# ArjunTeh/AdjointNonlinearRayTracing

Measured on AMD Instinct MI355X. Metric: ray-steps/sec (fwd+adjoint), 256^3 RIF grid, 1M rays x 512 steps, higher is better.
Workload: dtype f32

## Files before the change

### adjointnonlinearraytracing_amd/_lib.py

```python
from __future__ import annotations

import ctypes as C
import os
from typing import Optional

_HERE = os.path.dirname(os.path.abspath(__file__))
LIB_PATH = os.environ.get("DRRT_HIP_LIB") or os.path.join(_HERE, "libdrrt_hip.so")

FLAG_NONE = 0
FLAG_SORT_RAYS = 1
FLAG_CORRECTED_H = 2
FLAG_NO_ZERO = 4
FLAG_DIRECT_ATOMICS = 8
FLAG_DEBUG_COUNTERS = 16
FLAG_PAIR_GRID = 64
FLAG_PAIR_REUSE = 128
FLAG_QUAD_GRID, FLAG_QUAD_REUSE = FLAG_PAIR_GRID, FLAG_PAIR_REUSE
FLAG_Q16_POS_ONLY = 0x200000
FLAG_STATIC_WINDOW = 0x400000
FLAG_CHORD_KEY = 0x800000
FLAG_RING_WINDOW = 0x1000000
FLAG_DISPATCH_IN_ORDER = 0x2000000
FLAG_RING_SPARSE, FLAG_RING_GENERAL, FLAG_RING_DIRECT = 0x4000000, 0x8000000, 0x10000000
ADAM_MASK_BOUNDARY, ADAM_CLAMP_MIN = 1, 2

ERR_RES_MISMATCH, ERR_BAD_RES, ERR_ARG, ERR_HIP = -1, -2, -3, -4


class Stats(C.Structure):
    _fields_ = [("ray_steps", C.c_ulonglong), ("n_failed", C.c_ulonglong),
                ("iters", C.c_uint), ("reserved", C.c_uint)]


STATS_BYTES = C.sizeof(Stats)

_vp, _f, _sz, _u, _ll, _i = C.c_void_p, C.c_float, C.c_size_t, C.c_uint, C.c_longlong, C.c_int
_d = C.c_double
_tail = [_vp, _vp, _sz, _u, _vp]


def _sensor_signatures():
    e = [_vp, _f]
    splat = ([_i, _f, _vp, _u, _vp], [_i, _f, _vp, _vp, _vp, _vp])
    families = {
        "splat": ([_sz, _vp, _vp] + e, 4) + splat,
        "far_splat": ([_sz, _vp] + e, 2) + splat,
        "tex_get": ([_sz, _vp, _vp], 4, [_vp, _i, _f, _i, _vp, _vp], [_vp, _i, _f, _i, _vp, _vp, _vp, _vp]),
    }
    return {f"drrt_sensor_{family}{dframe}{bwd}_f32": (_i, rays + [_vp] * (1 if dframe else host) + tails[bool(bwd)])
            for family, (rays, host, *tails) in families.items() for dframe in ("", "_dframe") for bwd in ("", "_bwd")}


SIGNATURES = {
    "drrt_workspace_bytes": (_sz, [_sz, _u]),
    "drrt_workspace_bytes_grid": (_sz, [_sz, _ll, _u]),
    "drrt_last_error": (C.c_char_p, []),
    "drrt_version": (C.c_char_p, []),
    "drrt_trace_f32": (_i, [_vp, _ll, _vp, _sz, _vp, _vp, _f, _f, _vp, _vp] + _tail),
    "drrt_trace_f16io": (_i, [_vp, _ll, _vp, _sz, _vp, _vp, _f, _f, _vp, _vp] + _tail),
    "drrt_backtrace_f16io": (_i, [_vp, _ll, _vp, _sz, _vp, _vp, _vp, _vp, _f, _f, _vp] + _tail),
    "drrt_trace_q16io": (_i, [_vp, _ll, _vp, _sz, _vp, _vp, _f, _f, _vp, _vp] + _tail),
    "drrt_backtrace_q16io": (_i, [_vp, _ll, _vp, _sz, _vp, _vp, _vp, _vp, _f, _f, _vp] + _tail),
    "drrt_q16_params": (_i, [_vp, _f, _vp]),
    "drrt_q16_encode": (_i, [_vp, _f, _sz, _vp, _vp, _vp, _vp, _vp]),
    "drrt_q16_decode": (_i, [_vp, _f, _sz, _vp, _vp, _vp, _vp, _vp]),
    "drrt_trace_pln_f32": (_i, [_vp, _ll, _vp, _sz, _vp, _vp, _vp, _vp, _f, _f, _vp, _vp, _vp] + _tail),
    "drrt_trace_target_f32": (_i, [_vp, _ll, _vp, _sz, _vp, _vp, _vp, _f, _f, _vp, _vp, _vp] + _tail),
    "drrt_trace_sdf_f32": (_i, [_vp, _vp, _ll, _vp, _sz, _vp, _vp, _f, _f, _vp, _vp] + _tail),
    "drrt_trace_cable_f32": (_i, [_vp, _sz, _f, _f, _sz, _vp, _vp, _vp, _f, _vp, _vp, _vp] + _tail),
    "drrt_backtrace_f32": (_i, [_vp, _ll, _vp, _sz, _vp, _vp, _vp, _vp, _f, _f, _vp] + _tail),
    "drrt_backtrace_rays_f32": (_i, [_vp, _ll, _vp, _sz, _vp, _vp, _vp, _vp, _vp, _vp, _vp, _f, _f, _vp, _vp] + _tail),
    "drrt_trace_opl_f32": (_i, [_vp, _ll, _vp, _sz, _vp, _vp, _f, _f, _vp, _vp, _vp, _vp] + _tail),
    "drrt_backtrace_opl_f32": (_i, [_vp, _ll, _vp, _sz, _vp, _vp, _vp, _vp, _vp, _vp, _vp, _vp, _f, _f, _vp, _vp, _vp] + _tail),
    "drrt_trace_field_f32": (_i, [_vp, _vp, _ll, _vp, _sz, _vp, _vp, _f, _f, _vp, _vp, _vp, _vp] + _tail),
    "drrt_backtrace_field_f32": (_i, [_vp, _vp, _ll, _vp, _sz, _vp, _vp, _vp, _vp, _vp, _vp, _vp, _vp, _f, _f, _vp, _vp, _vp, _vp] + _tail),
    "drrt_trace_emission_f32": (_i, [_vp, _vp, _vp, _ll, _vp, _sz, _vp, _vp, _f, _f, _vp, _vp, _vp, _vp, _vp] + _tail),
    "drrt_backtrace_emission_f32": (_i, [_vp, _vp, _vp, _ll, _vp, _sz, _vp, _vp, _vp, _vp, _vp, _vp, _vp, _vp, _vp, _vp, _f, _f,
                                         _vp, _vp, _vp, _vp, _vp] + _tail),
    "drrt_backtrace_chunk_state_bytes": (_sz, [_sz]),
    "drrt_backtrace_max_steps": (_i, [_vp, _f, _f]),
    "drrt_backtrace_chunk_f32": (_i, [_vp, _ll, _vp, _sz, _vp, _vp, _vp, _vp, _f, _f, _vp] + _tail + [_vp, _sz, _i, _i, _vp]),
    "drrt_backtrace_sdf_f32": (_i, [_vp, _vp, _ll, _vp, _sz, _vp, _vp, _vp, _vp, _f, _f, _vp] + _tail),
    "drrt_backtrace_cable_f32": (_i, [_vp, _sz, _f, _f, _sz, _vp, _vp, _vp, _vp, _f, _vp] + _tail),
    "drrt_backtrace_cable_rays_f32": (_i, [_vp, _sz, _f, _f, _sz, _vp, _vp, _vp, _vp, _vp, _f, _vp, _vp] + _tail),
    "drrt_backtrace_pln_rays_f32": (_i, [_vp, _ll, _vp, _sz, _vp, _vp, _vp, _vp, _vp, _vp, _f, _f, _vp, _vp] + _tail),
    "drrt_backtrace_sdf_rays_f32": (_i, [_vp, _vp, _ll, _vp, _sz, _vp, _vp, _vp, _vp, _f, _f, _vp, _vp] + _tail),
    "drrt_backtrace_target_rays_f32": (_i, [_vp, _ll, _vp, _sz, _vp, _vp, _vp, _vp, _vp, _vp, _f, _f, _vp, _vp] + _tail),
    **_sensor_signatures(),
    "drrt_rays_to_plane_f32": (_i, [_sz, _vp, _vp, _vp, _vp, _i, _vp, _vp]),
    "drrt_rays_to_plane_bwd_f32": (_i, [_sz, _vp, _vp, _vp, _vp, _i, _vp, _vp, _vp, _vp]),
    "drrt_upres_volume_f32": (_i, [_vp, _vp, _vp, _vp, _vp]),
    "drrt_adam_step_f32": (_i, [_vp, _vp, _vp, _vp, _vp, _d, _d, _d, _d, _d, _d, _d, _u, _vp]),
    "drrt_gen_workspace_bytes": (_sz, [_i, _i, _i, _i]),
    "drrt_gen_rays_f32": (_i, [_i, _vp, _vp, _i, _i, _i, _i, _d, _d, _i, _i, _vp, _d, _vp, _vp, _vp, _vp, _vp, _sz, _vp]),
    "drrt_gen_cone_rays_f32": (_i, [_vp, _vp, _i, _i, _i, _i, _d, _d, _d, _vp, _d, _vp, _vp, _vp, _vp, _vp, _sz, _vp]),
    "drrt_last_order": (_vp, [_vp]),
    "drrt_set_order_hint": (None, [_vp, _sz]),
    "drrt_order_hint_pending": (_sz, []),
    "drrt_last_steps": (_vp, [_vp]),
    "drrt_set_step_hint": (None, [_vp, _sz]),
    "drrt_last_bundle_counters": (_vp, []),
    "drrt_ring_threshold_pct": (_i, []),
    "drrt_ring_long_threshold_permille": (_i, []),
    "drrt_ring_direct_threshold_pct": (_i, []),
    "drrt_profile_begin": (_i, [_i]),
    "drrt_profile_collect": (_i, [_vp, _vp, _i]),
    "drrt_profile_end": (None, []),
}

PROF_NAMES = {1: "trace", 2: "backtrace", 3: "sort", 4: "zero", 5: "quad", 6: "backtrace_rays",
              7: "backtrace_cable_rays", 8: "backtrace_pln_rays", 9: "backtrace_sdf_rays", 10: "backtrace_target_rays",
              11: "trace_opl", 12: "backtrace_opl", 13: "trace_field", 14: "backtrace_field"}
PROF_NAMES_MORE = {15: "trace_emission", 16: "backtrace_emission"}

_lib: Optional[C.CDLL] = None


def load() -> C.CDLL:
    global _lib
    if _lib is not None:
        return _lib
    if not os.path.exists(LIB_PATH):
        raise RuntimeError(
            f"libdrrt_hip.so not found at {LIB_PATH}: build it with "
            "`python -c 'import __graft_entry__ as g; g.build()'` or "
            "`make -C adjointnonlinearraytracing_amd/csrc`.  There is no CPU fallback.")
    import torch
    lib = C.CDLL(LIB_PATH)
    for name, (res, args) in SIGNATURES.items():
        fn = getattr(lib, name)
        fn.restype, fn.argtypes = res, args
    _lib = lib
    return lib


def profile_collect(max_out: int = 4096):
    ids = (C.c_int * max_out)()
    ms = (C.c_float * max_out)()
    n = load().drrt_profile_collect(ids, ms, max_out)
    return [(PROF_NAMES.get(ids[i]) or PROF_NAMES_MORE.get(ids[i], str(ids[i])), float(ms[i])) for i in range(n)]


def last_error() -> str:
    return load().drrt_last_error().decode()


def _p(t) -> C.c_void_p:
    return C.c_void_p(0 if t is None else t.data_ptr())


def _stream(device) -> C.c_void_p:
    import torch
    return C.c_void_p(torch.cuda.current_stream(device).cuda_stream)


def check(rc: int) -> None:
    if rc != 0:
        raise RuntimeError(last_error() or f"drrt_hip error {rc}")
```

### adjointnonlinearraytracing_amd/csrc/drrt_sort.hip

```cpp
#include <hip/hip_runtime.h>
#include <hip/hip_fp16.h>
#include <rocprim/device/device_radix_sort.hpp>
#include <stdint.h>

#include "drrt_device.h"
#include "drrt_keys.h"

namespace drrt {

__device__ __forceinline__ float ldr(const Vol& V, const void* p, size_t k, int io, bool is_pos) {
  if (io == 3) return is_pos ? q16_pos_dec(V, ((const uint16_t*)p)[k]) : ((const float*)p)[k];
  if (io == 2) return is_pos ? q16_pos_dec(V, ((const uint16_t*)p)[k]) : q16_vel_dec(((const int16_t*)p)[k]);
  return io ? __half2float(((const __half*)p)[k]) : ((const float*)p)[k];
}

__global__ void __launch_bounds__(256) k_chord_keys(Vol V, size_t n, const void* __restrict__ pos,
                                                    const void* __restrict__ vel, int io_half, float dir_sign,
                                                    uint64_t* __restrict__ keys, uint32_t* __restrict__ idx) {
  size_t i = (size_t)blockIdx.x * 256 + threadIdx.x;
  if (i >= n) return;
  float p[3] = {ldr(V, pos, 3 * i, io_half, true), ldr(V, pos, 3 * i + 1, io_half, true), ldr(V, pos, 3 * i + 2, io_half, true)};
  float d[3] = {dir_sign * ldr(V, vel, 3 * i, io_half, false), dir_sign * ldr(V, vel, 3 * i + 1, io_half, false),
                dir_sign * ldr(V, vel, 3 * i + 2, io_half, false)};
  keys[i] = chord_key(V, p, d);
  idx[i] = (uint32_t)i;
}

__global__ void __launch_bounds__(256) k_lightfield_keys(Vol V, size_t n, const void* __restrict__ pos,
                                                         const void* __restrict__ vel, int io_half, float dir_sign,
                                                         uint32_t* __restrict__ keys, uint32_t* __restrict__ idx) {
  size_t i = (size_t)blockIdx.x * 256 + threadIdx.x;
  if (i >= n) return;
  const float p[3] = {ldr(V, pos, 3 * i, io_half, true), ldr(V, pos, 3 * i + 1, io_half, true), ldr(V, pos, 3 * i + 2, io_half, true)};
  float d[3] = {dir_sign * ldr(V, vel, 3 * i, io_half, false), dir_sign * ldr(V, vel, 3 * i + 1, io_half, false),
                dir_sign * ldr(V, vel, 3 * i + 2, io_half, false)};
  idx[i] = (uint32_t)i;
  keys[i] = lightfield_key(V, p, d);
}

static inline size_t al(size_t v) { return (v + 255) / 256 * 256; }

static size_t radix_temp_bytes(size_t n) {
  size_t t64 = 0, t32 = 0;
  hipError_t e = rocprim::radix_sort_pairs(nullptr, t64, (const uint64_t*)nullptr, (uint64_t*)nullptr,
                                          (const uint32_t*)nullptr, (uint32_t*)nullptr, n, 0u, (unsigned)kKeyBits,
                                          (hipStream_t)0);
  hipError_t e2 = rocprim::radix_sort_pairs(nullptr, t32, (const uint32_t*)nullptr, (uint32_t*)nullptr,
                                           (const uint32_t*)nullptr, (uint32_t*)nullptr, n, 0u, (unsigned)kLfKeyBits,
                                           (hipStream_t)0);
  size_t temp = t64 > t32 ? t64 : t32;
  if (e != hipSuccess || e2 != hipSuccess || temp == 0) {
    (void)hipGetLastError();
    temp = n * 32 + (1u << 20);
  }
  return temp;
}

size_t sort_workspace_bytes(size_t n) {
  return 2 * al(n * sizeof(uint64_t)) + 2 * al(n * sizeof(uint32_t)) + al(radix_temp_bytes(n));
}

hipError_t sort_rays_by_entry_voxel(const Vol& V, float h, size_t n, const void* pos, const void* vel, int io_half,
                                    float dir_sign, void* ws, size_t ws_bytes, const uint32_t** perm_out,
                                    hipStream_t stream, bool chord_key) {
  (void)h;
  char* base = (char*)ws;
  const size_t k8 = al(n * sizeof(uint64_t)), k4 = al(n * sizeof(uint32_t));
  uint64_t* keys_in = (uint64_t*)(base);
  uint64_t* keys_out = (uint64_t*)(base + k8);
  uint32_t* idx_in = (uint32_t*)(base + 2 * k8);
  uint32_t* idx_out = (uint32_t*)(base + 2 * k8 + k4);
  void* temp = base + 2 * k8 + 2 * k4;
  size_t temp_bytes = ws_bytes - (2 * k8 + 2 * k4);
  hipError_t e;
  if (chord_key) {
    hipLaunchKernelGGL(k_chord_keys, dim3((unsigned)((n + 255) / 256)), dim3(256), 0, stream, V, n, pos, vel,
                       io_half, dir_sign, keys_in, idx_in);
    e = hipGetLastError();
    if (e != hipSuccess) return e;
    e = rocprim::radix_sort_pairs(temp, temp_bytes, (const uint64_t*)keys_in, keys_out,
                                  (const uint32_t*)idx_in, idx_out, n, 0u, (unsigned)kKeyBits, stream);
  } else {
    hipLaunchKernelGGL(k_lightfield_keys, dim3((unsigned)((n + 255) / 256)), dim3(256), 0, stream, V, n, pos, vel,
                       io_half, dir_sign, (uint32_t*)keys_in, idx_in);
    e = hipGetLastError();
    if (e != hipSuccess) return e;
    e = rocprim::radix_sort_pairs(temp, temp_bytes, (const uint32_t*)keys_in, (uint32_t*)keys_out,
                                  (const uint32_t*)idx_in, idx_out, n, 0u, (unsigned)kLfKeyBits, stream);
  }
  *perm_out = idx_out;
  return e;
}

}
```

### include/drrt_hip.h

```cpp
#ifndef DRRT_HIP_H
#define DRRT_HIP_H

#include <stddef.h>
#include <stdint.h>

#ifdef __cplusplus
extern "C" {
#endif

#if defined(__GNUC__)
#define DRRT_API __attribute__((visibility("default")))
#else
#define DRRT_API
#endif

#define DRRT_OK                0
#define DRRT_ERR_RES_MISMATCH (-1)
#define DRRT_ERR_BAD_RES      (-2)
#define DRRT_ERR_ARG          (-3)
#define DRRT_ERR_HIP          (-4)

#define DRRT_FLAG_NONE         0u
#define DRRT_FLAG_SORT_RAYS    1u
#define DRRT_FLAG_CORRECTED_H  2u
#define DRRT_FLAG_NO_ZERO      4u
#define DRRT_FLAG_DIRECT_ATOMICS 8u

#define DRRT_FLAG_PAIR_GRID    64u
#define DRRT_FLAG_PAIR_REUSE  128u
#define DRRT_FLAG_QUAD_GRID  DRRT_FLAG_PAIR_GRID
#define DRRT_FLAG_QUAD_REUSE DRRT_FLAG_PAIR_REUSE
#define DRRT_FLAG_Q16_POS_ONLY 0x200000u
#define DRRT_FLAG_CHORD_KEY 0x800000u
#define DRRT_FLAG_RING_WINDOW 0x1000000u
#define DRRT_FLAG_RING_SPARSE  0x4000000u
#define DRRT_FLAG_RING_GENERAL 0x8000000u
#define DRRT_FLAG_RING_DIRECT  0x10000000u
#define DRRT_FLAG_STATIC_WINDOW 0x400000u
#define DRRT_FLAG_DISPATCH_IN_ORDER 0x2000000u
#define DRRT_FLAG_DEBUG_COUNTERS 16u


typedef struct drrt_stats {
  unsigned long long ray_steps;
  unsigned long long n_failed;
  unsigned int       iters;
  unsigned int       reserved;
} drrt_stats;

DRRT_API size_t drrt_workspace_bytes(size_t n, unsigned flags);
DRRT_API size_t drrt_workspace_bytes_grid(size_t n, long long nvox, unsigned flags);

DRRT_API const char* drrt_last_error(void);

DRRT_API const char* drrt_version(void);

DRRT_API const uint32_t* drrt_last_order(size_t* n_out);
DRRT_API void drrt_set_order_hint(const uint32_t* order, size_t n);
DRRT_API size_t drrt_order_hint_pending(void);
DRRT_API const uint32_t* drrt_last_steps(size_t* n_out);
DRRT_API void drrt_set_step_hint(const uint32_t* steps, size_t n);

DRRT_API const unsigned* drrt_last_bundle_counters(void);
DRRT_API int drrt_ring_threshold_pct(void);
DRRT_API int drrt_ring_long_threshold_permille(void);
DRRT_API int drrt_ring_direct_threshold_pct(void);

DRRT_API int drrt_q16_params(const int res[3], float h, float out[3]);
DRRT_API int drrt_q16_encode(const int res[3], float h, size_t n, const float* pos, const float* vel,
                    void* pos_q, void* vel_q, void* stream);
DRRT_API int drrt_q16_decode(const int res[3], float h, size_t n, const void* pos_q, const void* vel_q,
                    float* pos, float* vel, void* stream);
DRRT_API int drrt_trace_q16io(const float* rif, long long nvox, const int res[3], size_t n,
                     const void* pos_q, const void* vel_q, float h, float ds,
                     void* xt_q, void* vt_q,
                     drrt_stats* stats, void* workspace, size_t workspace_bytes,
                     unsigned flags, void* stream);
DRRT_API int drrt_backtrace_q16io(const float* rif, long long nvox, const int res[3], size_t n,
                         const void* xt_q, const void* vt_q, const void* dx_h, const void* dv_h,
                         float h, float ds, float* grad,
                         drrt_stats* stats, void* workspace, size_t workspace_bytes,
                         unsigned flags, void* stream);


DRRT_API int drrt_trace_f32(const float* rif, long long nvox, const int res[3], size_t n,
                   const float* pos, const float* vel, float h, float ds,
                   float* xt, float* vt,
                   drrt_stats* stats, void* workspace, size_t workspace_bytes,
                   unsigned flags, void* stream);

DRRT_API int drrt_trace_f16io(const float* rif, long long nvox, const int res[3], size_t n,
                     const void* pos_h, const void* vel_h, float h, float ds,
                     void* xt_h, void* vt_h,
                     drrt_stats* stats, void* workspace, size_t workspace_bytes,
                     unsigned flags, void* stream);

DRRT_API int drrt_trace_pln_f32(const float* rif, long long nvox, const int res[3], size_t n,
                       const float* pos, const float* vel,
                       const float* pln_o, const float* pln_d, float h, float ds,
                       float* xt, float* vt, uint8_t* failmask,
                       drrt_stats* stats, void* workspace, size_t workspace_bytes,
                       unsigned flags, void* stream);

DRRT_API int drrt_trace_target_f32(const float* rif, long long nvox, const int res[3], size_t n,
                          const float* pos, const float* vel, const float* target,
                          float h, float ds, float* xt, float* vt, float* dist2,
                          drrt_stats* stats, void* workspace, size_t workspace_bytes,
                          unsigned flags, void* stream);

DRRT_API int drrt_trace_sdf_f32(const float* rif, const float* sdf, long long nvox, const int res[3],
                       size_t n, const float* pos, const float* vel, float h, float ds,
                       float* xt, float* vt,
                       drrt_stats* stats, void* workspace, size_t workspace_bytes,
                       unsigned flags, void* stream);

DRRT_API int drrt_trace_cable_f32(const float* rif, size_t rres, float radius, float length, size_t n,
                         const float* pos, const float* vel, const float* target, float ds,
                         float* xt, float* vt, float* dist2,
                         drrt_stats* stats, void* workspace, size_t workspace_bytes,
                         unsigned flags, void* stream);


DRRT_API int drrt_backtrace_f32(const float* rif, long long nvox, const int res[3], size_t n,
                       const float* xt, const float* vt, const float* dx, const float* dv,
                       float h, float ds, float* grad,
                       drrt_stats* stats, void* workspace, size_t workspace_bytes,
                       unsigned flags, void* stream);

DRRT_API int drrt_backtrace_rays_f32(const float* rif, long long nvox, const int res[3], size_t n,
                       const float* pos, const float* vel,
                       const float* xt, const float* vt,
                       const uint32_t* fwd_steps,
                       const float* dx, const float* dv, float h, float ds,
                       float* dpos, float* dvel,
                       drrt_stats* stats, void* workspace, size_t workspace_bytes,
                       unsigned flags, void* stream);

DRRT_API int drrt_trace_opl_f32(const float* rif, long long nvox, const int res[3], size_t n,
                       const float* pos, const float* vel, float h, float ds,
                       float* xt, float* vt, float* opl, uint32_t* steps_out,
                       drrt_stats* stats, void* workspace, size_t workspace_bytes,
                       unsigned flags, void* stream);

DRRT_API int drrt_backtrace_opl_f32(const float* rif, long long nvox, const int res[3], size_t n,
                       const float* pos, const float* vel,
                       const float* xt, const float* vt,
                       const uint32_t* fwd_steps,
                       const float* dx, const float* dv, const float* dopl, float h, float ds,
                       float* grad, float* dpos, float* dvel,
                       drrt_stats* stats, void* workspace, size_t workspace_bytes,
                       unsigned flags, void* stream);

DRRT_API int drrt_trace_field_f32(const float* rif, const float* field, long long nvox, const int res[3], size_t n,
                       const float* pos, const float* vel, float h, float ds,
                       float* xt, float* vt, float* tau, uint32_t* steps_out,
                       drrt_stats* stats, void* workspace, size_t workspace_bytes,
                       unsigned flags, void* stream);

DRRT_API int drrt_backtrace_field_f32(const float* rif, const float* field, long long nvox, const int res[3], size_t n,
                       const float* pos, const float* vel,
                       const float* xt, const float* vt,
                       const uint32_t* fwd_steps,
                       const float* dx, const float* dv, const float* dtau, float h, float ds,
                       float* grad, float* grad_field, float* dpos, float* dvel,
                       drrt_stats* stats, void* workspace, size_t workspace_bytes,
                       unsigned flags, void* stream);

DRRT_API int drrt_trace_emission_f32(const float* rif, const float* emission, const float* absorption, long long nvox,
                       const int res[3], size_t n,
                       const float* pos, const float* vel, float h, float ds,
                       float* xt, float* vt, float* rad, float* tau, uint32_t* steps_out,
                       drrt_stats* stats, void* workspace, size_t workspace_bytes,
                       unsigned flags, void* stream);

DRRT_API int drrt_backtrace_emission_f32(const float* rif, const float* emission, const float* absorption, long long nvox,
                       const int res[3], size_t n,
                       const float* pos, const float* vel,
                       const float* xt, const float* vt,
                       const uint32_t* fwd_steps, const float* tau,
                       const float* dx, const float* dv, const float* drad, const float* dtau, float h, float ds,
                       float* grad, float* grad_emission, float* grad_absorption, float* dpos, float* dvel,
                       drrt_stats* stats, void* workspace, size_t workspace_bytes,
                       unsigned flags, void* stream);

DRRT_API int drrt_backtrace_f16io(const float* rif, long long nvox, const int res[3], size_t n,
                         const void* xt_h, const void* vt_h, const void* dx_h, const void* dv_h,
                         float h, float ds, float* grad,
                         drrt_stats* stats, void* workspace, size_t workspace_bytes,
                         unsigned flags, void* stream);

DRRT_API size_t drrt_backtrace_chunk_state_bytes(size_t n);
DRRT_API int drrt_backtrace_max_steps(const int res[3], float h, float ds);
DRRT_API int drrt_backtrace_chunk_f32(const float* rif, long long nvox, const int res[3], size_t n,
                         const float* xt, const float* vt, const float* dx, const float* dv,
                         float h, float ds, float* grad,
                         drrt_stats* stats, void* workspace, size_t workspace_bytes,
                         unsigned flags, void* stream,
                         void* state, size_t state_bytes, int it_begin, int it_count, int* progress);

DRRT_API int drrt_backtrace_sdf_f32(const float* rif, const float* sdf, long long nvox, const int res[3],
                           size_t n, const float* xt, const float* vt,
                           const float* dx, const float* dv, float h, float ds, float* grad,
                           drrt_stats* stats, void* workspace, size_t workspace_bytes,
                           unsigned flags, void* stream);

DRRT_API int drrt_backtrace_cable_f32(const float* rif, size_t rres, float radius, float length, size_t n,
                             const float* xt, const float* vt, const float* dx, const float* dv,
                             float ds, float* grad,
                             drrt_stats* stats, void* workspace, size_t workspace_bytes,
                             unsigned flags, void* stream);

DRRT_API int drrt_backtrace_cable_rays_f32(const float* rif, size_t rres, float radius, float length, size_t n,
                             const float* pos, const float* vel, const float* target,
                             const float* dx, const float* dv, float ds,
                             float* dpos, float* dvel,
                             drrt_stats* stats, void* workspace, size_t workspace_bytes,
                             unsigned flags, void* stream);

DRRT_API int drrt_backtrace_pln_rays_f32(const float* rif, long long nvox, const int res[3], size_t n,
                             const float* pos, const float* vel, const float* pln_o, const float* pln_d,
                             const float* dx, const float* dv, float h, float ds,
                             float* dpos, float* dvel,
                             drrt_stats* stats, void* workspace, size_t workspace_bytes,
                             unsigned flags, void* stream);
DRRT_API int drrt_backtrace_sdf_rays_f32(const float* rif, const float* sdf, long long nvox, const int res[3], size_t n,
                             const float* pos, const float* vel,
                             const float* dx, const float* dv, float h, float ds,
                             float* dpos, float* dvel,
                             drrt_stats* stats, void* workspace, size_t workspace_bytes,
                             unsigned flags, void* stream);

DRRT_API int drrt_backtrace_target_rays_f32(const float* rif, long long nvox, const int res[3], size_t n,
                             const float* pos, const float* vel, const float* target,
                             const float* dx, const float* dv, const float* ddist2 ,
                             float h, float ds, float* dpos, float* dvel,
                             drrt_stats* stats, void* workspace, size_t workspace_bytes,
                             unsigned flags, void* stream);

DRRT_API int drrt_sensor_splat_f32(size_t n, const float* x, const float* v, const float* e, float e_scalar,
                          const float plane_p[3], const float plane_n[3], const float t1[3], const float t2[3],
                          int res, float span, float* image, unsigned flags, void* stream);
DRRT_API int drrt_sensor_splat_bwd_f32(size_t n, const float* x, const float* v, const float* e, float e_scalar,
                              const float plane_p[3], const float plane_n[3], const float t1[3], const float t2[3],
                              int res, float span, const float* grad_image, float* grad_x, float* grad_v,
                              void* stream);

DRRT_API int drrt_sensor_far_splat_f32(size_t n, const float* v, const float* e, float e_scalar, const float t1[3],
                              const float t2[3], int res, float ang_cut, float* image, unsigned flags, void* stream);
DRRT_API int drrt_sensor_far_splat_bwd_f32(size_t n, const float* v, const float* e, float e_scalar, const float t1[3],
                                  const float t2[3], int res, float ang_cut, const float* grad_image,
                                  float* grad_x, float* grad_v, void* stream);

DRRT_API int drrt_sensor_tex_get_f32(size_t n, const float* x, const float* v, const float plane_p[3], const float plane_n[3],
                            const float t1[3], const float t2[3], const float* tex, int res, float span, int mode,
                            float* f_out, void* stream);
DRRT_API int drrt_sensor_tex_get_bwd_f32(size_t n, const float* x, const float* v, const float plane_p[3],
                                const float plane_n[3], const float t1[3], const float t2[3], const float* tex, int res,
                                float span, int mode, const float* grad_f, float* grad_x, float* grad_v, void* stream);

DRRT_API int drrt_sensor_splat_dframe_f32(size_t n, const float* x, const float* v, const float* e, float e_scalar,
                                 const float* frame12, int res, float span, float* image, unsigned flags, void* stream);
DRRT_API int drrt_sensor_splat_dframe_bwd_f32(size_t n, const float* x, const float* v, const float* e, float e_scalar,
                                     const float* frame12, int res, float span, const float* grad_image, float* grad_x,
                                     float* grad_v, void* stream);
DRRT_API int drrt_sensor_far_splat_dframe_f32(size_t n, const float* v, const float* e, float e_scalar, const float* frame12,
                                     int res, float ang_cut, float* image, unsigned flags, void* stream);
DRRT_API int drrt_sensor_far_splat_dframe_bwd_f32(size_t n, const float* v, const float* e, float e_scalar,
                                         const float* frame12, int res, float ang_cut, const float* grad_image,
                                         float* grad_x, float* grad_v, void* stream);
DRRT_API int drrt_sensor_tex_get_dframe_f32(size_t n, const float* x, const float* v, const float* frame12, const float* tex,
                                   int res, float span, int mode, float* f_out, void* stream);
DRRT_API int drrt_sensor_tex_get_dframe_bwd_f32(size_t n, const float* x, const float* v, const float* frame12,
                                       const float* tex, int res, float span, int mode, const float* grad_f,
                                       float* grad_x, float* grad_v, void* stream);

DRRT_API int drrt_rays_to_plane_f32(size_t n, const float* x, const float* v, const float* plane_p, const float* plane_n,
                           int plane_stride, float* x_out, void* stream);
DRRT_API int drrt_rays_to_plane_bwd_f32(size_t n, const float* x, const float* v, const float* plane_p, const float* plane_n,
                               int plane_stride, const float* grad_x_out, float* grad_x, float* grad_v, void* stream);

DRRT_API int drrt_upres_volume_f32(const float* src, const int src_shape[3], float* dst, const int dst_shape[3],
                          void* stream);

#define DRRT_ADAM_MASK_BOUNDARY 1u
#define DRRT_ADAM_CLAMP_MIN     2u
DRRT_API int drrt_adam_step_f32(float* param, float* grad, float* exp_avg, float* exp_avg_sq, const int shape[3],
                       double step, double lr, double beta1, double beta2, double eps, double weight_decay,
                       double clamp_min, unsigned flags, void* stream);

#define DRRT_SOURCE_PLANE 0
#define DRRT_SOURCE_POINT 1
DRRT_API size_t drrt_gen_workspace_bytes(int n_views, int spp, int p0, int p1);
DRRT_API int drrt_gen_rays_f32(int kind, const float* u, const float* view_rot, int n_views, int spp, int p0, int p1,
                      double width, double sensor_dist, int circle, int independent,
                      const float* ic_rot, double span, float* x, float* v, float* planes,
                      int* view_counts, void* workspace, size_t workspace_bytes, void* stream);
DRRT_API int drrt_gen_cone_rays_f32(const float* u, const float* view_rot, int n_views, int spp, int p0, int p1,
                           double width, double sensor_dist, double cone_cos, const float* ic_rot_host, double span,
                           float* x, float* v, float* planes, int* view_counts, void* workspace,
                           size_t workspace_bytes, void* stream);

#define DRRT_PROF_TRACE      1
#define DRRT_PROF_BACKTRACE  2
#define DRRT_PROF_SORT       3
#define DRRT_PROF_ZERO       4
#define DRRT_PROF_QUAD       5
#define DRRT_PROF_BACKTRACE_RAYS 6
#define DRRT_PROF_BACKTRACE_CABLE_RAYS 7
#define DRRT_PROF_BACKTRACE_PLN_RAYS 8
#define DRRT_PROF_BACKTRACE_SDF_RAYS 9
#define DRRT_PROF_BACKTRACE_TARGET_RAYS 10
#define DRRT_PROF_TRACE_OPL 11
#define DRRT_PROF_BACKTRACE_OPL 12
#define DRRT_PROF_TRACE_FIELD 13
#define DRRT_PROF_BACKTRACE_FIELD 14
#define DRRT_PROF_TRACE_EMISSION 15
#define DRRT_PROF_BACKTRACE_EMISSION 16
DRRT_API int  drrt_profile_begin(int capacity);
DRRT_API int  drrt_profile_collect(int* kernel_ids, float* ms, int max_out);
DRRT_API void drrt_profile_end(void);

#ifdef __cplusplus
}
#endif
#endif
```

Baseline: 93.28 billion.

## Replace rocprim radix sort with custom three-pass lightfield radix sort

```diff
diff --git a/adjointnonlinearraytracing_amd/_lib.py b/adjointnonlinearraytracing_amd/_lib.py
--- a/adjointnonlinearraytracing_amd/_lib.py
+++ b/adjointnonlinearraytracing_amd/_lib.py
@@ -103,6 +103,8 @@
     "drrt_ring_threshold_pct": (_i, []),
     "drrt_ring_long_threshold_permille": (_i, []),
     "drrt_ring_direct_threshold_pct": (_i, []),
+    "drrt_sort_radix_min_rays": (_i, []),
+    "drrt_sort_radix_max_rays": (_i, []),
     "drrt_profile_begin": (_i, [_i]),
     "drrt_profile_collect": (_i, [_vp, _vp, _i]),
     "drrt_profile_end": (None, []),
diff --git a/adjointnonlinearraytracing_amd/csrc/drrt_sort.hip b/adjointnonlinearraytracing_amd/csrc/drrt_sort.hip
--- a/adjointnonlinearraytracing_amd/csrc/drrt_sort.hip
+++ b/adjointnonlinearraytracing_amd/csrc/drrt_sort.hip
@@ -1,8 +1,11 @@
 #include <hip/hip_runtime.h>
 #include <hip/hip_fp16.h>
+#include <rocprim/block/block_radix_sort.hpp>
+#include <rocprim/block/block_scan.hpp>
 #include <rocprim/device/device_radix_sort.hpp>
 #include <stdint.h>
 
+#include "../../include/drrt_hip.h"
 #include "drrt_device.h"
 #include "drrt_keys.h"
 
@@ -26,16 +29,196 @@
   idx[i] = (uint32_t)i;
 }
 
+__device__ __forceinline__ uint32_t ray_lightfield_key(const Vol& V, size_t i, const void* __restrict__ pos,
+                                                       const void* __restrict__ vel, int io_half, float dir_sign) {
+  const float p[3] = {ldr(V, pos, 3 * i, io_half, true), ldr(V, pos, 3 * i + 1, io_half, true), ldr(V, pos, 3 * i + 2, io_half, true)};
+  float d[3] = {dir_sign * ldr(V, vel, 3 * i, io_half, false), dir_sign * ldr(V, vel, 3 * i + 1, io_half, false),
+                dir_sign * ldr(V, vel, 3 * i + 2, io_half, false)};
+  return lightfield_key(V, p, d);
+}
+
 __global__ void __launch_bounds__(256) k_lightfield_keys(Vol V, size_t n, const void* __restrict__ pos,
                                                          const void* __restrict__ vel, int io_half, float dir_sign,
                                                          uint32_t* __restrict__ keys, uint32_t* __restrict__ idx) {
   size_t i = (size_t)blockIdx.x * 256 + threadIdx.x;
   if (i >= n) return;
-  const float p[3] = {ldr(V, pos, 3 * i, io_half, true), ldr(V, pos, 3 * i + 1, io_half, true), ldr(V, pos, 3 * i + 2, io_half, true)};
-  float d[3] = {dir_sign * ldr(V, vel, 3 * i, io_half, false), dir_sign * ldr(V, vel, 3 * i + 1, io_half, false),
-                dir_sign * ldr(V, vel, 3 * i + 2, io_half, false)};
   idx[i] = (uint32_t)i;
-  keys[i] = lightfield_key(V, p, d);
+  keys[i] = ray_lightfield_key(V, i, pos, vel, io_half, dir_sign);
+}
+
+#ifndef DRRT_SORT_RADIX_ITEMS
+#define DRRT_SORT_RADIX_ITEMS 4
+#endif
+constexpr int kRxItems = DRRT_SORT_RADIX_ITEMS;
+constexpr int kRxTile = 256 * kRxItems, kRxPosBits = kRxItems == 4 ? 10 : 11, kRxMaxDigitBits = 11;
+constexpr int kRxScanDigits = 16, kRxScanChunks = 16;
+#ifndef DRRT_SORT_RADIX_MIN_RAYS
+#define DRRT_SORT_RADIX_MIN_RAYS 262144
+#endif
+#ifndef DRRT_SORT_RADIX_MAX_RAYS
+#define DRRT_SORT_RADIX_MAX_RAYS (1 << 21)
+#endif
+
+template <int SHIFT, int BITS, bool FIRST>
+__global__ void __launch_bounds__(256) k_radix_hist(Vol V, uint32_t n, const void* __restrict__ pos,
+                                                    const void* __restrict__ vel, int io_half, float dir_sign,
+                                                    uint32_t* __restrict__ keys, uint32_t* __restrict__ table) {
+  constexpr uint32_t ND = 1u << BITS;
+  __shared__ uint32_t cnt[ND];
+  for (uint32_t d = threadIdx.x; d < ND; d += 256) cnt[d] = 0;
+  __syncthreads();
+  const uint32_t base = blockIdx.x * (uint32_t)kRxTile + threadIdx.x;
+#pragma unroll 4
+  for (int k = 0; k < kRxItems; ++k) {
+    const uint32_t i = base + (uint32_t)k * 256u;
+    if (i < n) {
+      uint32_t key;
+      if (FIRST) { key = ray_lightfield_key(V, i, pos, vel, io_half, dir_sign); keys[i] = key; }
+      else key = keys[i];
+      atomicAdd(&cnt[(key >> SHIFT) & (ND - 1u)], 1u);
+    }
+  }
+  __syncthreads();
+  for (uint32_t d = threadIdx.x; d < ND; d += 256) table[blockIdx.x * ND + d] = cnt[d];
+}
+
+template <int BITS>
+__global__ void __launch_bounds__(256) k_radix_scan(uint32_t* __restrict__ table, uint32_t* __restrict__ totals,
+                                                    uint32_t ntiles) {
+  constexpr uint32_t ND = 1u << BITS;
+  static_assert(ND % kRxScanDigits == 0, "a scan block takes 16 digits");
+  __shared__ uint32_t part[kRxScanChunks][kRxScanDigits + 1];
+  const uint32_t dl = threadIdx.x % kRxScanDigits, c = threadIdx.x / kRxScanDigits;
+  const uint32_t d = blockIdx.x * kRxScanDigits + dl;
+  const uint32_t per = (ntiles + kRxScanChunks - 1) / kRxScanChunks;
+  const uint32_t t0 = c * per < ntiles ? c * per : ntiles, t1 = t0 + per < ntiles ? t0 + per : ntiles;
+  uint32_t sum = 0;
+#pragma unroll 8
+  for (uint32_t t = t0; t < t1; ++t) sum += table[t * ND + d];
+  part[c][dl] = sum;
+  __syncthreads();
+  uint32_t run = 0, tot = 0;
+#pragma unroll
+  for (uint32_t j = 0; j < (uint32_t)kRxScanChunks; ++j) {
+    const uint32_t v = part[j][dl];
+    run += j < c ? v : 0u;
+    tot += v;
+  }
+  if (c == 0) totals[d] = tot;
+#pragma unroll 8
+  for (uint32_t t = t0; t < t1; ++t) {
+    const uint32_t v = table[t * ND + d];
+    table[t * ND + d] = run;
+    run += v;
+  }
+}
+
+template <int SHIFT, int BITS, bool FIRST, bool LAST>
+__global__ void __launch_bounds__(256) k_radix_scatter(uint32_t n, const uint32_t* __restrict__ keys_in,
+                                                       const uint32_t* __restrict__ idx_in,
+                                                       uint32_t* __restrict__ keys_out, uint32_t* __restrict__ idx_out,
+                                                       const uint32_t* __restrict__ table,
+                                                       const uint32_t* __restrict__ totals) {
+  constexpr uint32_t ND = 1u << BITS, DPT = ND / 256u, POS = (1u << kRxPosBits) - 1u;
+  static_assert(ND >= 256u && kRxItems % 4 == 0 && (1 << kRxPosBits) == kRxTile, "tile shape");
+  using Sort = rocprim::block_radix_sort<uint32_t, 256, kRxItems>;
+  using Scan = rocprim::block_scan<uint32_t, 256>;
+  struct Rank { uint32_t comb[ND]; uint32_t tail[256]; typename Scan::storage_type scan; };
+  __shared__ union { typename Sort::storage_type sort; Rank r; } sm;
+  static_assert(sizeof(sm) <= 16384, "at most 16 KiB of LDS per block");
+
+  const uint32_t tid = threadIdx.x, base = blockIdx.x * (uint32_t)kRxTile, p0 = tid * (uint32_t)kRxItems;
+  uint32_t pk[kRxItems];
+  if (base + p0 + kRxItems <= n) {
+    uint32_t kk[kRxItems];
+#pragma unroll
+    for (int k = 0; k < kRxItems; k += 4) {
+      const uint4 a = *(const uint4*)(keys_in + base + p0 + k);
+      kk[k] = a.x; kk[k + 1] = a.y; kk[k + 2] = a.z; kk[k + 3] = a.w;
+    }
+#pragma unroll
+    for (int k = 0; k < kRxItems; ++k) pk[k] = (((kk[k] >> SHIFT) & (ND - 1u)) << kRxPosBits) | (p0 + k);
+  } else {
+#pragma unroll
+    for (int k = 0; k < kRxItems; ++k) {
+      const uint32_t i = base + p0 + k;
+      const uint32_t dg = i < n ? (keys_in[i] >> SHIFT) & (ND - 1u) : ND;
+      pk[k] = (dg << kRxPosBits) | (p0 + k);
+    }
+  }
+  uint32_t tot[DPT], row[DPT];
+#pragma unroll
+  for (uint32_t k = 0; k < DPT; ++k) { tot[k] = totals[tid * DPT + k]; row[k] = table[blockIdx.x * ND + tid * DPT + k]; }
+
+  Sort().sort(pk, sm.sort, kRxPosBits, kRxPosBits + BITS + 1);
+  __syncthreads();
+  sm.r.tail[tid] = pk[kRxItems - 1];
+  __syncthreads();
+  uint32_t prev = tid ? sm.r.tail[tid - 1] >> kRxPosBits : 0xffffffffu;
+#pragma unroll
+  for (int k = 0; k < kRxItems; ++k) {
+    const uint32_t dg = pk[k] >> kRxPosBits;
+    if (dg != prev && dg < ND) sm.r.comb[dg] = p0 + k;
+    prev = dg;
+  }
+  uint32_t mine = 0, ex = 0;
+#pragma unroll
+  for (uint32_t k = 0; k < DPT; ++k) mine += tot[k];
+  Scan().exclusive_scan(mine, ex, 0u, sm.r.scan);
+  __syncthreads();
+#pragma unroll
+  for (uint32_t k = 0; k < DPT; ++k) {
+    const uint32_t dg = tid * DPT + k;
+    sm.r.comb[dg] = ex + row[k] - sm.r.comb[dg];
+    ex += tot[k];
+  }
+  __syncthreads();
+#pragma unroll
+  for (int k = 0; k < kRxItems; ++k) {
+    const uint32_t dg = pk[k] >> kRxPosBits;
+    if (dg < ND) {
+      const uint32_t dst = sm.r.comb[dg] + p0 + k, src = base + (pk[k] & POS);
+      if (dst < n) {
+        if (!LAST) keys_out[dst] = keys_in[src];
+        idx_out[dst] = FIRST ? src : idx_in[src];
+      }
+    }
+  }
+}
+
+template <int SHIFT, int BITS, bool FIRST, bool LAST>
+static hipError_t radix_pass(const Vol& V, uint32_t n, const void* pos, const void* vel, int io_half, float dir_sign,
+                             uint32_t* keys_in, const uint32_t* idx_in, uint32_t* keys_out, uint32_t* idx_out,
+                             uint32_t* table, uint32_t* totals, hipStream_t stream) {
+  const uint32_t ntiles = (n + kRxTile - 1) / kRxTile;
+  hipLaunchKernelGGL((k_radix_hist<SHIFT, BITS, FIRST>), dim3(ntiles), dim3(256), 0, stream, V, n, pos, vel, io_half,
+                     dir_sign, keys_in, table);
+  hipLaunchKernelGGL((k_radix_scan<BITS>), dim3((1u << BITS) / kRxScanDigits), dim3(256), 0, stream, table, totals, ntiles);
+  hipLaunchKernelGGL((k_radix_scatter<SHIFT, BITS, FIRST, LAST>), dim3(ntiles), dim3(256), 0, stream, n,
+                     (const uint32_t*)keys_in, idx_in, keys_out, idx_out, (const uint32_t*)table, (const uint32_t*)totals);
+  return hipGetLastError();
+}
+
+static size_t radix_table_bytes(size_t n) {
+  return ((n + kRxTile - 1) / kRxTile) * ((size_t)1 << kRxMaxDigitBits) * sizeof(uint32_t);
+}
+static bool radix_qualifies(size_t n, const void* temp, size_t temp_bytes) {
+  static_assert(kLfKeyBits == 32 && 2 * kPosBits == 22, "the three passes below cut the key 11 + 11 + 10");
+  return n >= (size_t)DRRT_SORT_RADIX_MIN_RAYS && n <= (size_t)DRRT_SORT_RADIX_MAX_RAYS && (uintptr_t)temp % 16 == 0 &&
+         temp_bytes >= radix_table_bytes(n) + ((size_t)1 << kRxMaxDigitBits) * sizeof(uint32_t);
+}
+
+static hipError_t radix_sort_lightfield(const Vol& V, size_t n_, const void* pos, const void* vel, int io_half,
+                                        float dir_sign, uint32_t* k_a, uint32_t* k_b, uint32_t* i_a, uint32_t* i_b,
+                                        void* temp, hipStream_t stream) {
+  const uint32_t n = (uint32_t)n_;
+  uint32_t* table = (uint32_t*)temp;
+  uint32_t* totals = (uint32_t*)((char*)temp + radix_table_bytes(n_));
+  hipError_t e = radix_pass<0, 11, true, false>(V, n, pos, vel, io_half, dir_sign, k_a, nullptr, k_b, i_b, table, totals, stream);
+  if (e != hipSuccess) return e;
+  e = radix_pass<11, 11, false, false>(V, n, pos, vel, io_half, dir_sign, k_b, i_b, k_a, i_a, table, totals, stream);
+  if (e != hipSuccess) return e;
+  return radix_pass<22, 10, false, true>(V, n, pos, vel, io_half, dir_sign, k_a, i_a, nullptr, i_b, table, totals, stream);
 }
 
 static inline size_t al(size_t v) { return (v + 255) / 256 * 256; }
@@ -80,6 +263,10 @@
     if (e != hipSuccess) return e;
     e = rocprim::radix_sort_pairs(temp, temp_bytes, (const uint64_t*)keys_in, keys_out,
                                   (const uint32_t*)idx_in, idx_out, n, 0u, (unsigned)kKeyBits, stream);
+  } else if (n >= (size_t)DRRT_SORT_RADIX_MIN_RAYS && n <= (size_t)DRRT_SORT_RADIX_MAX_RAYS &&
+             radix_qualifies(n, temp, temp_bytes < al(radix_temp_bytes(n)) ? temp_bytes : al(radix_temp_bytes(n)))) {
+    e = radix_sort_lightfield(V, n, pos, vel, io_half, dir_sign, (uint32_t*)keys_in, (uint32_t*)keys_out, idx_in, idx_out,
+                              temp, stream);
   } else {
     hipLaunchKernelGGL(k_lightfield_keys, dim3((unsigned)((n + 255) / 256)), dim3(256), 0, stream, V, n, pos, vel,
                        io_half, dir_sign, (uint32_t*)keys_in, idx_in);
@@ -93,3 +280,6 @@
 }
 
 }
+
+extern "C" int drrt_sort_radix_min_rays(void) { return DRRT_SORT_RADIX_MIN_RAYS; }
+extern "C" int drrt_sort_radix_max_rays(void) { return DRRT_SORT_RADIX_MAX_RAYS; }
diff --git a/include/drrt_hip.h b/include/drrt_hip.h
--- a/include/drrt_hip.h
+++ b/include/drrt_hip.h
@@ -65,6 +65,9 @@
 DRRT_API int drrt_ring_threshold_pct(void);
 DRRT_API int drrt_ring_long_threshold_permille(void);
 DRRT_API int drrt_ring_direct_threshold_pct(void);
+
+DRRT_API int drrt_sort_radix_min_rays(void);
+DRRT_API int drrt_sort_radix_max_rays(void);
 
 DRRT_API int drrt_q16_params(const int res[3], float h, float out[3]);
 DRRT_API int drrt_q16_encode(const int res[3], float h, size_t n, const float* pos, const float* vel,
```

Result: no change. 93.99 billion, median of 5 (+0.8%).
